# ZongyueQin/SessionSimilaritySearch

Hardware: AMD Instinct MI355X
Metric: session queries/sec (higher is better)
Workload: dtype f32

## Files before the change

sessionsimilaritysearch_amd/_lib.py:

```python
from __future__ import annotations

import ctypes
import os
import subprocess
from ctypes import c_float, c_int, c_int32, c_int64, c_size_t, c_void_p

_HERE = os.path.dirname(os.path.abspath(__file__))
LIB_PATH = os.path.join(_HERE, "libsss.so")
CSRC = os.path.join(_HERE, "csrc")

_lib = None

_SIGNATURES = {
    "sss_version": (c_int, []),
    "sss_last_error": (ctypes.c_char_p, []),
    "sss_normalize_rows": (c_int, [c_void_p, c_int64, c_int, c_int64, c_float, c_int, c_void_p]),
    "sss_row_norm_max": (c_int, [c_void_p, c_int64, c_int, c_int, c_void_p, c_void_p]),
    "sss_f32_to_bf16": (c_int, [c_void_p, c_int64, c_void_p, c_void_p]),
    "sss_ip_topk_workspace_bytes": (c_size_t, [c_int64, c_int64, c_int, c_int, c_int]),
    "sss_ip_topk_state_bytes": (c_size_t, [c_int64]),
    "sss_ip_topk": (c_int, [c_void_p, c_int64, c_void_p, c_int64, c_int, c_int, c_int, c_int64, c_float,
                            c_void_p, c_void_p, c_void_p, c_void_p, c_void_p, c_size_t, c_void_p, c_size_t, c_void_p]),
    "sss_split_bf16": (c_int, [c_void_p, c_int64, c_int, c_void_p, c_void_p]),
    "sss_ip_topk_split": (c_int, [c_void_p, c_int64, c_void_p, c_void_p, c_int64, c_int, c_int, c_int64, c_float,
# ... 84 lines not shown
    "sss_sparse_topk_workspace_bytes": (c_size_t, [c_int64, c_int64]),
    "sss_sparse_topk": (c_int, [c_void_p, c_void_p, c_void_p, c_int64, c_void_p, c_void_p, c_void_p, c_int64, c_int, c_int64,
                                c_void_p, c_void_p, c_void_p, c_size_t, c_void_p]),
}

_L2_SIGNATURES = {
    "sss_l2_row_bias": (c_int, [c_void_p, c_int64, c_int, c_void_p, c_void_p]),
    "sss_l2_topk_workspace_bytes": (c_size_t, [c_int64, c_int64, c_int, c_int, c_int]),
    "sss_l2_topk": (c_int, [c_void_p, c_int64, c_void_p, c_void_p, c_int, c_int, c_float, c_void_p, c_int64, c_int, c_int, c_int64,
                            c_float, c_void_p, c_void_p, c_void_p, c_void_p, c_void_p, c_size_t, c_void_p, c_size_t, c_void_p]),
    "sss_l2_topk_threshold_workspace_bytes": (c_size_t, [c_int64, c_int64, c_int, c_int]),
    "sss_l2_topk_threshold": (c_int, [c_void_p, c_void_p, c_int64, c_void_p, c_void_p, c_int, c_int, c_float, c_void_p, c_int64, c_int,
                                      c_int, c_int64, c_float, c_void_p, c_void_p, c_void_p, c_void_p, c_size_t, c_void_p]),
}


class LinearProblem(ctypes.Structure):
    _fields_ = [("x", c_void_p), ("ldx", c_int64), ("ids", c_void_p), ("table", c_void_p), ("xcopy", c_void_p),
                ("ld_xcopy", c_int64), ("w", c_void_p), ("ldw", c_int64), ("bias", c_void_p), ("y", c_void_p),
                ("ldy", c_int64), ("n", c_int64), ("m", c_int32), ("act", c_int32), ("post_scale", c_void_p), ("post_shift", c_void_p)]


class GraphOut(ctypes.Structure):
    _fields_ = [(n, c_void_p) for n in ("q_x", "q_batch", "q_pos", "p_x", "p_batch", "p_cnt", "rowptr_qp", "col_qp",
                                        "rowptr_pq", "col_pq", "rowptr_pp", "col_pp", "w_pp", "src_row", "pos_id")]


class LayerArgs(ctypes.Structure):
    _fields_ = [("yp", c_void_p), ("ld_yp", c_int64), ("yq", c_void_p), ("ld_yq", c_int64), ("h", c_int32), ("d_x", c_int32),
                ("rowptr_qp", c_void_p), ("col_qp", c_void_p), ("rowptr_pp", c_void_p), ("col_pp", c_void_p),
                ("w_pp", c_void_p), ("bias_qp", c_void_p), ("b_ih", c_void_p),
                ("xin_p", c_void_p), ("ld_xin", c_int64), ("out_p", c_void_p), ("ld_out_p", c_int64), ("np", c_int64),
                ("rowptr_pq", c_void_p), ("col_pq", c_void_p), ("bias_pq", c_void_p),
                ("out_q", c_void_p), ("ld_out_q", c_int64), ("nq", c_int64), ("n_self_loop", c_int64),
                ("row_p", c_void_p), ("row_q", c_void_p), ("x0_p", c_void_p), ("ld_x0_p", c_int64),
                ("xq_table", c_void_p), ("ld_xq", c_int64), ("x0_q", c_void_p), ("ld_x0_q", c_int64)]


def exported_symbols():
    return sorted(_SIGNATURES)


def sparse_symbols():
    return sorted(_SPARSE_SIGNATURES)


def l2_symbols():
    return sorted(_L2_SIGNATURES)


def build(verbose: bool = False) -> str:
    cmd = ["make", "-C", CSRC, "-j4"]
    res = subprocess.run(cmd, capture_output=True, text=True)
    if res.returncode != 0:
        raise RuntimeError("building libsss.so failed:\n" + res.stdout[-4000:] + res.stderr[-4000:])
    if verbose:
        print(res.stdout)
    return LIB_PATH


def lib():
    global _lib
    if _lib is None:
        if not os.path.exists(LIB_PATH):
            raise RuntimeError(
                f"{LIB_PATH} is missing: the HIP extension is not built. Run "
                "`python -c 'import __graft_entry__ as g; g.build()'` (or `make -C "
                "sessionsimilaritysearch_amd/csrc`). There is no CPU fallback.")
        h = ctypes.CDLL(LIB_PATH)
        for name, (res, args) in (*_SIGNATURES.items(), *_SPARSE_SIGNATURES.items(), *_L2_SIGNATURES.items()):
            fn = getattr(h, name)
            fn.restype, fn.argtypes = res, args
        _lib = h
    return _lib


class SssError(RuntimeError):
    pass


def check(rc: int, what: str):
    if rc != 0:
        msg = lib().sss_last_error()
        raise SssError(f"{what} failed (rc={rc}): {msg.decode() if msg else ''}")

# ... 16 lines not shown
```

sessionsimilaritysearch_amd/csrc/capi.hip:

```cpp
#include <stdarg.h>
#include <stdio.h>

#include <mutex>
#include <set>
#include <utility>

#include "../../include/sss.h"
#include "../../include/sss_sparse.h"
#include "../../include/sss_l2.h"
#include "sss_common.h"
#include "scan.h"
#include "kargs.h"

namespace sss {

static thread_local char g_err[512] = "";

void set_error(const char* fmt, ...) {
    va_list ap;
    va_start(ap, fmt);
    vsnprintf(g_err, sizeof(g_err), fmt, ap);
    va_end(ap);
}

// ... 34 lines not shown
int gather_concat_rows(const float*, const long*, int, const float*, long, int, int, long, float*, long, hipStream_t);
int linear_f32(const float*, long, const float*, long, const float*, float*, long, long, int, int, hipStream_t);
int gat_aggregate(const float*, long, const float*, long, const float*, long, const int*, const int*, long, int,
                  const float*, int, long, float*, long, hipStream_t);
int csr_weighted_sum(const float*, long, const int*, const int*, const float*, long, int, float*, long, hipStream_t);
int gru_combine(const float*, long, const float*, long, const float*, long, int, const float*, long, long, int,
                float*, long, hipStream_t);
int pool_expand(const float*, const float*, long, const int*, const int*, long, long, int, int, const float*, float*,
                long, hipStream_t);
int segment_pool(const float*, long, const int*, const int*, long, long, int, const float*, long, const float*, long,
                 const float*, float*, long, hipStream_t);
int segment_ptr(const long*, long, long, int*, hipStream_t);

int linear_grouped(LinBatch&, hipStream_t);
int layer_update(const LayerArgs&, hipStream_t);
int pool_expand_mean(const float*, const float*, long, const int*, const int*, const int*, const int*, long, long, int, int,
                     const float*, float*, long, float*, long, hipStream_t);
int pool_attention(const float*, long, const float*, long, const float*, long, const float*, const int*, const int*, long, long,
                   int, int, float, int, float*, long, hipStream_t);
int pool_attention_tab(const float*, long, const float*, long, const float*, const float*, const float*, const float*, const int*,
                       const int*, const int*, const int*, long, long, long, int, int, int, float, float*, long, hipStream_t);
int csr_mean(const float*, long, const int*, const int*, long, int, float*, long, hipStream_t);
int segment_reduce(const float*, long, const float*, const int*, long, int, int, float*, long, hipStream_t);
int attention_dot_pool(const float*, long, const int*, long, int, float*, long, hipStream_t);
int item_vote(const float*, const long*, long, int, const long*, const int*, long, long, int, long*, double*, int*, hipStream_t);
size_t hamming_workspace_bytes(long nq, long n);
int hamming_capacity(long nq, long n);
int hamming_topk(const unsigned char*, long, const unsigned char*, long, int, int, long, int*, long*, int*, void*, size_t, hipStream_t);
size_t hamming_exhaustive_workspace_bytes(long nsel, long n);
int hamming_topk_exhaustive(const unsigned char*, const int*, long, const unsigned char*, long, int, int, long, int*, long*, void*,
// ... 186 lines not shown
    sss::LinBatch b;
    b.nprob = n_problems; b.K = k;
    for (int i = 0; i < n_problems; ++i) {
        const sss_linear_problem& s = problems[i];
        sss::LinProb& p = b.p[i];
        p.x = s.x; p.ldx = s.ldx; p.ids = reinterpret_cast<const long*>(s.ids); p.table = s.table; p.xcopy = s.xcopy;
        p.ld_xcopy = s.ld_xcopy; p.w = s.w; p.ldw = s.ldw; p.bias = s.bias; p.y = s.y; p.ldy = s.ldy; p.n = s.n; p.m = s.m;
        p.act = s.act; p.post_scale = s.post_scale; p.post_shift = s.post_shift; p.tiles_m = 0; p.tile_begin = 0;
        if (s.act < 0 || s.act > 4 || (s.post_scale == nullptr) != (s.post_shift == nullptr)) {
            sss::set_error("linear_grouped: problem %d: act must be 0..4, post_scale / post_shift come together", i);
            return SSS_EINVAL;
        }
    }
    return sss::linear_grouped(b, ST(stream));
}
int sss_hetero_layer_update(const sss_layer_args* a, void* stream) {
    if (!a) { sss::set_error("hetero_layer_update: null args"); return SSS_EINVAL; }
    sss::LayerArgs l;
    l.Yp = a->yp; l.ldyp = a->ld_yp; l.Yq = a->yq; l.ldyq = a->ld_yq; l.h = a->h; l.d_x = a->d_x;
    l.rowptr_qp = a->rowptr_qp; l.col_qp = a->col_qp; l.rowptr_pp = a->rowptr_pp; l.col_pp = a->col_pp; l.w_pp = a->w_pp;
    l.bias_qp = a->bias_qp; l.b_ih = a->b_ih; l.xin_p = a->xin_p; l.ld_xin = a->ld_xin; l.out_p = a->out_p;
    l.ld_outp = a->ld_out_p; l.Np = a->np; l.rowptr_pq = a->rowptr_pq; l.col_pq = a->col_pq; l.bias_pq = a->bias_pq;
    l.out_q = a->out_q; l.ld_outq = a->ld_out_q; l.Nq = a->nq; l.n_self_loop = a->n_self_loop;
    l.row_p = reinterpret_cast<const long*>(a->row_p); l.row_q = reinterpret_cast<const long*>(a->row_q);
    l.x0_p = a->x0_p; l.ld_x0p = a->ld_x0_p; l.xq_table = a->xq_table; l.ld_xq = a->ld_xq; l.x0_q = a->x0_q; l.ld_x0q = a->ld_x0_q;
    return sss::layer_update(l, ST(stream));
}
int sss_pool_expand_mean(const float* lin_p, const float* lin_q, int64_t ld_lin, const int32_t* src_row,
                         const int32_t* pos_id, const int32_t* pptr, const int32_t* qptr, int64_t n_clicks,
                         int64_t n_graphs, int d_lin, int p, const float* pos_emb, float* node, int64_t ld_node,
                         float* coarse, int64_t ld_coarse, void* stream) {
    return sss::pool_expand_mean(lin_p, lin_q, ld_lin, src_row, pos_id, pptr, qptr, n_clicks, n_graphs, d_lin, p, pos_emb,
                                 node, ld_node, coarse, ld_coarse, ST(stream));
}
int sss_pool_attention(const float* node, int64_t ld_node, const float* a, int64_t ld_a, const float* b, int64_t ld_b,
                       const float* watt, const int32_t* pptr, const int32_t* qptr, int64_t n_clicks, int64_t n_graphs,
                       int d, int normalize, float eps, int reduce_sum, float* out, int64_t ld_out, void* stream) {
    return sss::pool_attention(node, ld_node, a, ld_a, b, ld_b, watt, pptr, qptr, n_clicks, n_graphs, d, normalize, eps,
                               reduce_sum, out, ld_out, ST(stream));
}
int sss_pool_attention_tab(const float* t, int64_t ld_t, const float* ac, int64_t ld_ac, const float* tanhpos, const float* a2tab,
// ... 50 lines not shown
    g.rowptr_qp = o->rowptr_qp; g.col_qp = o->col_qp; g.rowptr_pq = o->rowptr_pq; g.col_pq = o->col_pq;
    g.rowptr_pp = o->rowptr_pp; g.col_pp = o->col_pp; g.w_pp = o->w_pp; g.src_row = o->src_row; g.pos_id = o->pos_id;
    return sss::graph_fill(reinterpret_cast<const long*>(sess_ptr), is_search, reinterpret_cast<const long*>(item_id),
                           reinterpret_cast<const long*>(query_tok), n_sessions, bases, g, ST(stream));
}
int sss_knn_item_vote(const float* D, const int64_t* I, int64_t nq, int s, const int64_t* items_ptr, const int32_t* items,
                      int64_t id_offset, int64_t n_sessions, int k, int64_t* out_items, double* out_weights,
                      int32_t* status, void* stream) {
    return sss::item_vote(D, reinterpret_cast<const long*>(I), nq, s, reinterpret_cast<const long*>(items_ptr), items,
                          id_offset, n_sessions, k, reinterpret_cast<long*>(out_items), out_weights, status, ST(stream));
}
int sss_segment_ptr(const int64_t* batch, int64_t n, int64_t n_graphs, int32_t* ptr, void* stream) {
    return sss::segment_ptr(reinterpret_cast<const long*>(batch), n, n_graphs, ptr, ST(stream));
}

int sss_session_vectors_count(const int64_t* sess_ptr, const uint8_t* is_search, const int64_t* item_id, int64_t n_sessions,
                              int64_t n_items, int32_t* counts, int32_t* err, void* stream) {
    return sss::session_vectors_count(reinterpret_cast<const long*>(sess_ptr), is_search, reinterpret_cast<const long*>(item_id),
                                      n_sessions, n_items, counts, err, ST(stream));
}
int sss_session_vectors_fill(const int64_t* sess_ptr, const uint8_t* is_search, const int64_t* item_id, int64_t n_sessions,
                             int64_t n_items, int mode, double lammy, const int64_t* ptr, int32_t* items, float* weights,
                             int32_t* err, void* stream) {
    return sss::session_vectors_fill(reinterpret_cast<const long*>(sess_ptr), is_search, reinterpret_cast<const long*>(item_id),
                                     n_sessions, n_items, mode, lammy, reinterpret_cast<const long*>(ptr), items, weights, err,
                                     ST(stream));
}
size_t sss_sparse_topk_workspace_bytes(int64_t nq, int64_t n) { return sss::sparse_topk_workspace_bytes(nq, n); }
int sss_sparse_topk(const int64_t* q_ptr, const int32_t* q_items, const float* q_weights, int64_t nq, const int64_t* c_ptr,
                    const int32_t* c_items, const float* c_weights, int64_t n, int k, int64_t id_offset, float* D_out,
// ... 32 lines not shown
```

sessionsimilaritysearch_amd/csrc/gnn.hip:

```cpp
#include "sss_common.h"
#include "kargs.h"

namespace sss {

int normalize_rows(float* x, long n, int d, long ld, float eps, int rule, hipStream_t st);

constexpr int LT = 64;

int linear_grouped(LinBatch& b, hipStream_t st);

template <int LPR>
__global__ __launch_bounds__(256) void k_gat_aggregate(
    const float* __restrict__ xs, long ld_xs, const float* __restrict__ a_src, long ld_as,
    const float* __restrict__ a_dst, long ld_ad, const int* __restrict__ rowptr,
    const int* __restrict__ col, long n_dst, int h, const float* __restrict__ bias, int relu,
    long n_self_loop, float* __restrict__ out, long ld_out) {
    const int sub = threadIdx.x % LPR;
    const long per_block = 256 / LPR;
    const int nv = h / 4;
    auto score = [&](long j, float ad) {
        const float v = a_src[j * ld_as] + ad;
        return v > 0.f ? v : 0.2f * v;
    };
    for (long i = (long)blockIdx.x * per_block + threadIdx.x / LPR; i < n_dst; i += (long)gridDim.x * per_block) {
// ... 326 lines not shown
                                           out, ld_out));
    return check_launch("k_segment_pool");
}

int segment_ptr(const long* batch, long n, long n_graphs, int* ptr, hipStream_t st) {
    if (n < 0 || n_graphs < 0) { set_error("segment_ptr: bad arguments"); return SSS_EINVAL; }
    hipLaunchKernelGGL(k_segment_ptr, dim3((unsigned)((n_graphs + 1 + 255) / 256)), dim3(256), 0, st, batch, n, n_graphs, ptr);
    return check_launch("k_segment_ptr");
}

}

namespace sss {


template <int KC>
__global__ __launch_bounds__(256, 2) void k_linear_grouped(const LinBatch B) {
    constexpr int CPR = KC / 4;
    constexpr int NLD = LT * CPR / 256;
    constexpr int RS = CPR;
    constexpr int SW = RS < 16 ? RS - 1 : 15;
    extern __shared__ __attribute__((aligned(16))) float lds_raw[];
    float* lx = lds_raw;
    float* lw = lds_raw + LT * RS * 4;
    int pi = 0;
#pragma unroll
    for (int i = 1; i < 4; ++i)
        if (i < B.nprob && (int)blockIdx.x >= B.p[i].tile_begin) pi = i;
    const float* X = B.p[0].x; long ldx = B.p[0].ldx; const long* ids = B.p[0].ids; const float* table = B.p[0].table;
    float* xcopy = B.p[0].xcopy; long ldc = B.p[0].ld_xcopy; const float* W = B.p[0].w; long ldw = B.p[0].ldw;
    const float* bias = B.p[0].bias; float* Y = B.p[0].y; long ldy = B.p[0].ldy; long N = B.p[0].n; int M = B.p[0].m;
    int tiles_m = B.p[0].tiles_m, tile_begin = B.p[0].tile_begin, act = B.p[0].act;
    const float* post_s = B.p[0].post_scale; const float* post_t = B.p[0].post_shift;
#pragma unroll
    for (int i = 1; i < 4; ++i)
        if (pi == i) {
            act = B.p[i].act; post_s = B.p[i].post_scale; post_t = B.p[i].post_shift;
            X = B.p[i].x; ldx = B.p[i].ldx; ids = B.p[i].ids; table = B.p[i].table; xcopy = B.p[i].xcopy; ldc = B.p[i].ld_xcopy;
            W = B.p[i].w; ldw = B.p[i].ldw; bias = B.p[i].bias; Y = B.p[i].y; ldy = B.p[i].ldy; N = B.p[i].n; M = B.p[i].m;
            tiles_m = B.p[i].tiles_m; tile_begin = B.p[i].tile_begin;
        }
    const int K = B.K;
    const int t = (int)blockIdx.x - tile_begin;
    const long row0 = (long)(t / tiles_m) * LT;
    const int col0 = (t % tiles_m) * LT;
    const int tid = threadIdx.x, lane = tid & 63, wave = tid >> 6;
    const int wr = wave >> 1, wc = wave & 1;
    const int r = lane & 31, h = lane >> 5;
    const int xr = wr * 32 + r, wrow = wc * 32 + r;

    f32x16 acc = {0};
    f32x4 sx[NLD], sw[NLD];
    auto fetch = [&](int k0) {
#pragma unroll
        for (int i = 0; i < NLD; ++i) {
            const int p = tid + 256 * i;
            const int tr = p / CPR, c = p % CPR;
            long gr = row0 + tr; if (gr > N - 1) gr = N - 1;
            int gw = col0 + tr; if (gw > M - 1) gw = M - 1;
            const float* xrow = ids ? table + ids[gr] * (long)K : X + gr * ldx;
            sx[i] = *reinterpret_cast<const f32x4*>(xrow + k0 + c * 4);
// ... 35 lines not shown
    if (col < M) {
        const float bv = bias ? bias[col] : 0.f;
        const float ps = post_s ? post_s[col] : 1.f, pt = post_s ? post_t[col] : 0.f;
#pragma unroll
        for (int j = 0; j < 16; ++j) {
            const long row = row0 + wr * 32 + (j & 3) + 8 * (j >> 2) + 4 * h;
            float v = acc[j] + bv;
            if (act == 1) v = fmaxf(v, 0.f);
            else if (act == 2) v = tanhf(v);
            else if (act == 3) v = v > 0.f ? 1.f : v < 0.f ? -1.f : v;
            else if (act == 4) v = tanhf(tanhf(v));
            if (post_s) {
#pragma clang fp contract(off)
                v = fmaxf(v * ps + pt, 0.f);
            }
            if (row < N) Y[row * ldy + col] = v;
        }
    }
}


__device__ __forceinline__ float4 f4_fma(float w, float4 x, float4 a) {
    a.x += w * x.x; a.y += w * x.y; a.z += w * x.z; a.w += w * x.w;
    return a;
}
__device__ __forceinline__ float leaky02(float v) { return v > 0.f ? v : 0.2f * v; }

__device__ __forceinline__ float4 gat_row(const float* xs, long ld, const float* a_src_col, float ad, const int* col,
                                          int e0, int e1, int c4, const float* bias, long skip_i, long self_i,
                                          const long* row_of = nullptr) {
    float mx = -INFINITY, den = 0.f;
    float4 acc = make_float4(0.f, 0.f, 0.f, 0.f);
    auto edge = [&](long jn) {
// ... 7 lines not shown
        }
        const float ex = expf(v - mx);
        den += ex;
        acc = f4_fma(ex, x, acc);
    };
    for (int e = e0; e < e1; ++e) {
        const long j = col[e];
        if (j != skip_i) edge(j);
    }
    if (self_i >= 0) edge(self_i);
    const float inv = 1.f / (den + 1e-16f);
    const float4 b = *reinterpret_cast<const float4*>(bias + c4);
    return make_float4(acc.x * inv + b.x, acc.y * inv + b.y, acc.z * inv + b.z, acc.w * inv + b.w);
}

template <int LPR>
__global__ __launch_bounds__(256) void k_layer_update(const LayerArgs A) {
    const int sub = threadIdx.x % LPR;
    const long per_block = 256 / LPR;
    const long t = (long)blockIdx.x * per_block + threadIdx.x / LPR;
    const int h = A.h, c4 = sub * 4;
    if (c4 >= h || t >= A.Np + A.Nq) return;
    if (t >= A.Np) {
        const long i = t - A.Np;
        const long ri = A.row_q ? A.row_q[i] : i;
        const float ad = A.Yq[ri * A.ldyq + h + 1];
        const bool lp = i < A.n_self_loop;
        float4 o = gat_row(A.Yp, A.ldyp, A.Yp + 7 * h, ad, A.col_pq, A.rowptr_pq[i], A.rowptr_pq[i + 1], c4, A.bias_pq,
                           A.n_self_loop > 0 ? i : -1, lp ? i : -1, A.row_p);
        if (A.x0_q) {
            const float* xq = A.xq_table + ri * A.ld_xq;
            float* dq = A.x0_q + i * A.ld_x0q;
            if (c4 + 3 < A.d_x) *reinterpret_cast<float4*>(dq + c4) = *reinterpret_cast<const float4*>(xq + c4);
            else for (int u = 0; u < 4; ++u) if (c4 + u < A.d_x) dq[c4 + u] = xq[c4 + u];
        }
        o.x = fmaxf(o.x, 0.f); o.y = fmaxf(o.y, 0.f); o.z = fmaxf(o.z, 0.f); o.w = fmaxf(o.w, 0.f);
        *reinterpret_cast<float4*>(A.out_q + i * A.ld_outq + c4) = o;
// ... 34 lines not shown
            if (c4 + 1 < A.d_x) dp[c4 + 1] = xv.y;
            if (c4 + 2 < A.d_x) dp[c4 + 2] = xv.z;
        }
    }
    float4 o;
#define SSS_GRU1(f)                                                        \
    {                                                                      \
        const float rr = sigmoidf_(gr.f + hr.f);                           \
        const float zz = sigmoidf_(gz.f + hz.f);                           \
        const float nn = tanhf(gn.f + rr * hn.f);                          \
        o.f = fmaxf(t1.f + (1.f - zz) * nn + zz * xv.f, 0.f);              \
    }
    SSS_GRU1(x) SSS_GRU1(y) SSS_GRU1(z) SSS_GRU1(w)
#undef SSS_GRU1
    *reinterpret_cast<float4*>(A.out_p + i * A.ld_outp + c4) = o;
}

template <int LPR>
__global__ __launch_bounds__(256) void k_pool_expand_mean(const float* __restrict__ lin_p, const float* __restrict__ lin_q,
                                                          long ld_lin, const int* __restrict__ src_row,
                                                          const int* __restrict__ pos_id, const int* __restrict__ pptr,
                                                          const int* __restrict__ qptr, long n_clicks, long n_graphs,
                                                          int Dl, int P, const float* __restrict__ pos_emb,
                                                          float* __restrict__ node, long ld_node,
                                                          float* __restrict__ coarse, long ld_coarse) {
    const int sub = threadIdx.x % LPR;
    const long g = (long)blockIdx.x * (256 / LPR) + threadIdx.x / LPR;
    const int D = Dl + P, c4 = sub * 4;
    if (g >= n_graphs || c4 >= D) return;
    const int p0 = pptr[g], p1 = pptr[g + 1], q0 = qptr[g], q1 = qptr[g + 1];
// ... 186 lines not shown
            (p.ids && (!p.table || (p.xcopy && (p.ld_xcopy % 4 || p.ld_xcopy < b.K))))) {
            set_error("linear_grouped: problem %d has bad strides / shapes", i);
            return SSS_EINVAL;
        }
        p.tiles_m = (p.m + LT - 1) / LT;
        p.tile_begin = total;
        total += (int)((p.n + LT - 1) / LT) * p.tiles_m;
    }
    for (int i = b.nprob; i < 4; ++i) { b.p[i] = b.p[0]; b.p[i].tile_begin = 0x7fffffff; }
    if (total == 0) return SSS_OK;
    const int lds32 = 2 * LT * 8 * 16;
    hipLaunchKernelGGL(k_linear_grouped<32>, dim3((unsigned)total), dim3(256), lds32, st, b);
    return check_launch("k_linear_grouped");
}

int layer_update(const LayerArgs& a, hipStream_t st) {
    if (a.h <= 0 || a.h % 4 || a.h > 256 || a.Np < 0 || a.Nq < 0 || a.d_x > a.h || a.ldyp % 4 || a.ldyq % 4 || a.ld_outp % 4 ||
        a.ld_outq % 4 || (a.d_x >= 4 && a.ld_xin % 4) || a.ldyp < 7 * a.h + 2 || a.ldyq < a.h + 2) {
        set_error("layer_update: need h %% 4 == 0, h <= 256, d_x <= h, 16-byte aligned row strides, ldyp >= 7h+2, ldyq >= h+2");
        return SSS_EINVAL;
    }
    if ((a.x0_p && a.ld_x0p % 4) || (a.x0_q && (!a.xq_table || a.ld_xq % 4 || a.ld_x0q % 4))) {
        set_error("layer_update: x0_p / x0_q need 16-byte aligned row strides, x0_q needs xq_table");
        return SSS_EINVAL;
    }
    const long total = a.Np + a.Nq;
    if (total == 0) return SSS_OK;
    const int lpr = lanes_for(a.h);
    const long per = 256 / lpr;
    SSS_LPR_SWITCH(lpr, hipLaunchKernelGGL(k_layer_update<L>, dim3((unsigned)((total + per - 1) / per)), dim3(256), 0, st, a));
    return check_launch("k_layer_update");
}

int pool_expand_mean(const float* lin_p, const float* lin_q, long ld_lin, const int* src_row, const int* pos_id,
                     const int* pptr, const int* qptr, long n_clicks, long n_graphs, int Dl, int P, const float* pos_emb,
                     float* node, long ld_node, float* coarse, long ld_coarse, hipStream_t st) {
    const int D = Dl + P;
    if (n_graphs < 0 || Dl <= 0 || P < 0 || D % 4 || D > 256 || ld_node % 4 || ld_node < D || ld_coarse % 4 || ld_coarse < D) {
        set_error("pool_expand_mean: need (Dl + P) %% 4 == 0, <= 256, 16-byte aligned row strides");
        return SSS_EINVAL;
    }
    if (n_graphs == 0) return SSS_OK;
    const int lpr = lanes_for(D);
    const long per = 256 / lpr;
    SSS_LPR_SWITCH(lpr, hipLaunchKernelGGL(k_pool_expand_mean<L>, dim3((unsigned)((n_graphs + per - 1) / per)), dim3(256), 0, st,
                                           lin_p, lin_q, ld_lin, src_row, pos_id, pptr, qptr, n_clicks, n_graphs, Dl, P, pos_emb,
// ... 47 lines not shown
```

sessionsimilaritysearch_amd/csrc/kargs.h:

```cpp
#pragma once
#include "sss_common.h"

namespace sss {

struct LinProb {
    const float* x; long ldx;
    const long* ids; const float* table;
    float* xcopy; long ld_xcopy;
    const float* w; long ldw; const float* bias;
    float* y; long ldy;
    long n; int m;
    int act;
    const float* post_scale = nullptr;
    const float* post_shift = nullptr;
    int tiles_m, tile_begin;
};
struct LinBatch { LinProb p[4]; int nprob; int K; };

struct LayerArgs {
    const float* Yp; long ldyp; const float* Yq; long ldyq; int h;
    const int* rowptr_qp; const int* col_qp; const int* rowptr_pp; const int* col_pp; const float* w_pp;
    const float* bias_qp; const float* b_ih; const float* xin_p; long ld_xin; int d_x; float* out_p; long ld_outp; long Np;
    const int* rowptr_pq; const int* col_pq; const float* bias_pq; float* out_q; long ld_outq; long Nq;
    long n_self_loop;
    const long* row_p = nullptr; const long* row_q = nullptr;
    float* x0_p = nullptr; long ld_x0p = 0;
    const float* xq_table = nullptr; long ld_xq = 0; float* x0_q = nullptr; long ld_x0q = 0;
};

struct GraphOut {
    long* q_x; long* q_batch; int* q_pos;
    long* p_x; long* p_batch; long* p_cnt;
    int* rowptr_qp; int* col_qp;
    int* rowptr_pq; int* col_pq;
    int* rowptr_pp; int* col_pp; float* w_pp;
    int* src_row; int* pos_id;
};

}
```

sessionsimilaritysearch_amd/encoder.py:

```python
from __future__ import annotations

import ctypes
import itertools
import math
from dataclasses import dataclass

import numpy as np
import torch

from . import _lib
from .sessions import ASIN_NUM, EDGE_PP, EDGE_PQ, EDGE_QP, MAX_SEQ_LEN, QUERY_VOCAB, ActionTable

ALPHA_PAD = 32


@dataclass
class EncoderConfig:
    d_in: int = 128
    d_id: int = 0
    h: int = 128
    n_layers: int = 2
    d_out: int = 128
    max_seq_len: int = MAX_SEQ_LEN
    n_items: int = ASIN_NUM
# ... 94 lines not shown
    rowptr[1:] = torch.cumsum(counts, 0).to(torch.int32)
    wv = None if w is None else w[order].float().contiguous()
    return rowptr, col, wv


class PreparedBatch:
    """Device-resident batch: feature ids + CSR adjacencies + pooling index arrays
    (``SessionEncoder.prepare``)."""


class SessionEncoder:

    _serials = itertools.count()

    def __init__(self, cfg: EncoderConfig, weights: dict, device=None, use_edge_weight: bool = False,
                 debug_nan_checks: bool = False, fused: bool = True):
        cfg.validate()
        self._serial = next(SessionEncoder._serials)
        if not torch.cuda.is_available():
            raise _lib.SssError("no HIP device available: the encoder runs on MI355X only")
        _lib.lib()
        self.user_cfg = cfg
        self.d_id, self.d_feat = cfg.d_id, cfg.d_in
        if cfg.d_id:
            weights = self._internal_weights(cfg, weights)
            cfg = EncoderConfig(**{**cfg.__dict__, "d_in": cfg.d_p, "d_id": 0})
        self.cfg = cfg
        self.device = torch.device("cuda", torch.cuda.current_device()) if device is None else torch.device(device)
        self.use_edge_weight = use_edge_weight
        self.debug_nan_checks = debug_nan_checks
        self.fused = fused
        self.training = False
        self._prepare(weights)

    def eval(self):
        self.training = False
        return self

    def to(self, device):
        if torch.device(device) != self.device:
            raise _lib.SssError("SessionEncoder is bound to its construction device")
        return self

    def __call__(self, *a, **kw):
        return self.forward(*a, **kw)

# ... 267 lines not shown
                self._tabs = ()
            else:
                Yp = torch.empty((ni, 7 * h + ALPHA_PAD), dtype=torch.float32, device=self.device)
                Yq = torch.empty((nqy, h + ALPHA_PAD), dtype=torch.float32, device=self.device)
                P_ = _lib.LinearProblem
                mk = lambda x, w, b, y, n, m: P_(x=x.data_ptr(), ldx=x.stride(0), ids=0, table=0, xcopy=0, ld_xcopy=0,
                                                 w=w.data_ptr(), ldw=w.stride(0), bias=0 if b is None else b.data_ptr(),
                                                 y=y.data_ptr(), ldy=y.stride(0), n=n, m=m, act=0)
                arr = (P_ * 2)(mk(self.item_table, lw["w7"], lw["b7"], Yp, ni, 7 * h + 2),
                               mk(self.query_table, lw["wq"], None, Yq, nqy, h + 2))
                _lib.check(_lib.lib().sss_linear_grouped(arr, 2, lw["din"], self._st()), "sss_linear_grouped")
                self._tabs = (Yp, Yq)
        return self._tabs or None

    def _fused_calls(self, pb, ws, gather):
        key = "gather" if gather else "rows"
        if key in ws["calls"]:
            return ws["calls"][key]
        cfg = self.cfg
        h, D, P, W = cfg.h, cfg.d_out, cfg.max_seq_len, cfg.node_width
        NQ, NP, Yp, Yq = ws["NQ"], ws["NP"], ws["Yp"], ws["Yq"]
        P_ = _lib.LinearProblem

        def prob(x, w, bias, y, n, m, ids=None, table=None, xcopy=None):
            return P_(x=0 if x is None else x.data_ptr(), ldx=0 if x is None else x.stride(0),
                      ids=0 if ids is None else ids.data_ptr(), table=0 if table is None else table.data_ptr(),
                      xcopy=0 if xcopy is None else xcopy.data_ptr(), ld_xcopy=0 if xcopy is None else xcopy.stride(0),
                      w=w.data_ptr(), ldw=w.stride(0), bias=0 if bias is None else bias.data_ptr(),
                      y=y.data_ptr(), ldy=y.stride(0), n=n, m=m, act=0)

        steps, keep = [], []
# ... 28 lines not shown
                                np=pb.Np, rowptr_pq=rp_pq.data_ptr(), col_pq=c_pq.data_ptr(),
                                bias_pq=lw["bias_pq"].data_ptr(), out_q=out_q.data_ptr(), ld_out_q=NQ.stride(0), nq=pb.Nq,
                                n_self_loop=pb.n_self_loop,
                                row_p=pb.p_ids.data_ptr() if table0 else 0, row_q=pb.q_ids.data_ptr() if table0 else 0,
                                x0_p=NP.data_ptr() if table0 else 0, ld_x0_p=NP.stride(0),
                                xq_table=self.query_table.data_ptr() if table0 else 0,
                                ld_xq=self.query_table.stride(0) if table0 else 0,
                                x0_q=NQ.data_ptr() if table0 else 0, ld_x0_q=NQ.stride(0))
            if arr is not None:
                steps.append(("lin", arr, 2, din))
            steps.append(("layer", la))
            keep += [arr, la]
        pw, pt = self.pool, self.pool_tab
        Dl = D - P
        T, AC = ws["T"], ws["AC"]
        pp, pq = prob(NP, pw["wp"], pw["bp"], T[:pb.Np], pb.Np, Dl), prob(NQ, pw["wq"], pw["bq"], T[pb.Np:], pb.Nq, Dl)
        pp.act = pq.act = 2
        arr = (P_ * 2)(pp, pq)
        steps.append(("lin", arr, 2, W))
        arr2 = (P_ * 1)(prob(T, pt["wnc"], None, AC, pb.Np + pb.Nq, 2 * D))
        steps.append(("lin", arr2, 1, pt["KT"]))
        ws["calls"][key] = steps
        return steps

    def _forward_fused(self, pb, get_node, query_node_mask, product_node_mask, l2_normalize):
        cfg, L, dev = self.cfg, _lib.lib(), self.device
        h, D, P, W = cfg.h, cfg.d_out, cfg.max_seq_len, cfg.node_width
        ws = self._workspace(pb, get_node)
        NQ, NP = ws["NQ"], ws["NP"]
        masked = query_node_mask is not None or product_node_mask is not None
        gather = pb.q_feat is None and pb.p_feat is None and not masked
        if not gather:
            self._features(pb.q_ids, pb.q_feat, self.query_table, pb.Nq, NQ)
            self._features(pb.p_ids, pb.p_feat, self.item_table, pb.Np, NP, product=True)
            if query_node_mask is not None:
                NQ[:, :cfg.d_in] *= query_node_mask.to(dev, torch.float32).view(-1, 1)
            if product_node_mask is not None:
                NP[:, :cfg.d_in] *= product_node_mask.to(dev, torch.float32).view(-1, 1)
        elif self.item_table is None or self.query_table is None:
            raise _lib.SssError("no feature table in the weights and no .feat on the batch")
        st = self._st()
        pw = self.pool
        for step in self._fused_calls(pb, ws, gather):
            if step[0] == "lin":
                _lib.check(L.sss_linear_grouped(step[1], step[2], step[3], st), "sss_linear_grouped")
            else:
                _lib.check(L.sss_hetero_layer_update(ctypes.byref(step[1]), st), "sss_hetero_layer_update")
        out = torch.empty((pb.B, D), dtype=torch.float32, device=dev)
        pt, T, AC = self.pool_tab, ws["T"], ws["AC"]
        rc = L.sss_pool_attention_tab(T.data_ptr(), T.stride(0), AC.data_ptr(), AC.stride(0), pt["tanhpos"].data_ptr(),
                                      pt["a2"].data_ptr(), pt["c2"].data_ptr(), pw["watt"].data_ptr(), pb.src_row.data_ptr(),
                                      pb.pos_id.data_ptr(), pb.pptr.data_ptr(), pb.qptr.data_ptr(), pb.n_clicks, pb.Np, pb.B,
                                      D - P, P, 1 if l2_normalize else 0, 1e-6, out.data_ptr(), D, st)
        _lib.check(rc, "sss_pool_attention_tab")
        return out, NQ, NP

    @torch.no_grad()
    def forward(self, data, query_node_mask=None, product_node_mask=None, get_node=False, get_token=False,
                l2_normalize=False):
        cfg, L, dev = self.cfg, _lib.lib(), self.device
        h, D, P, W = cfg.h, cfg.d_out, cfg.max_seq_len, cfg.node_width
        pb = self.prepare(data)
# ... 90 lines not shown
```

Before: 487,200.

## Fuse last GNN layer update with pooling-head linear projections in one kernel

Adds a kernel that, per 64-row tile, runs the final hetero layer GRU update, then the per-type pooling projection (tanh) into T, then the wnc projection into AC, using 1024-thread blocks of four 256-thread teams. The three launches become one, and each tile's intermediates stay L2/LDS-local instead of round-tripping between launches. The linear tile body is refactored into a shared device function. The cost is fewer blocks (one per row tile), with teams idling when the column tile count isn't a multiple of four, and a smaller K chunk of 32, which could reduce GEMM efficiency.

```diff
diff --git a/include/sss_encoder.h b/include/sss_encoder.h
--- /dev/null
+++ b/include/sss_encoder.h
@@ -0,0 +1,22 @@
+#ifndef SSS_ENCODER_H
+#define SSS_ENCODER_H
+
+#include "sss.h"
+
+#ifdef __cplusplus
+extern "C" {
+#endif
+
+typedef struct {
+    const float* node_p; int64_t ld_np; const float* node_q; int64_t ld_nq; int32_t node_width;
+    const float* wp; int64_t ld_wp; const float* bp; const float* wq; int64_t ld_wq; const float* bq; int32_t d_lin;
+    float* t; int64_t ld_t; int32_t kt;
+    const float* wnc; int64_t ld_wnc; float* ac; int64_t ld_ac; int32_t m_ac;
+} sss_head_args;
+
+int sss_layer_update_head(const sss_layer_args* layer, const sss_head_args* head, void* stream);
+
+#ifdef __cplusplus
+}
+#endif
+#endif
diff --git a/sessionsimilaritysearch_amd/_lib.py b/sessionsimilaritysearch_amd/_lib.py
--- a/sessionsimilaritysearch_amd/_lib.py
+++ b/sessionsimilaritysearch_amd/_lib.py
@@ -122,6 +122,10 @@
                                       c_int, c_int64, c_float, c_void_p, c_void_p, c_void_p, c_void_p, c_size_t, c_void_p]),
 }
 
+_ENCODER_SIGNATURES = {
+    "sss_layer_update_head": (c_int, [c_void_p, c_void_p, c_void_p]),
+}
+
 
 class LinearProblem(ctypes.Structure):
     _fields_ = [("x", c_void_p), ("ldx", c_int64), ("ids", c_void_p), ("table", c_void_p), ("xcopy", c_void_p),
@@ -145,6 +149,13 @@
                 ("xq_table", c_void_p), ("ld_xq", c_int64), ("x0_q", c_void_p), ("ld_x0_q", c_int64)]
 
 
+class HeadArgs(ctypes.Structure):
+    _fields_ = [("node_p", c_void_p), ("ld_np", c_int64), ("node_q", c_void_p), ("ld_nq", c_int64), ("node_width", c_int32),
+                ("wp", c_void_p), ("ld_wp", c_int64), ("bp", c_void_p), ("wq", c_void_p), ("ld_wq", c_int64), ("bq", c_void_p),
+                ("d_lin", c_int32), ("t", c_void_p), ("ld_t", c_int64), ("kt", c_int32),
+                ("wnc", c_void_p), ("ld_wnc", c_int64), ("ac", c_void_p), ("ld_ac", c_int64), ("m_ac", c_int32)]
+
+
 def exported_symbols():
     return sorted(_SIGNATURES)
 
@@ -155,6 +166,10 @@
 
 def l2_symbols():
     return sorted(_L2_SIGNATURES)
+
+
+def encoder_symbols():
+    return sorted(_ENCODER_SIGNATURES)
 
 
 def build(verbose: bool = False) -> str:
@@ -176,7 +191,8 @@
                 "`python -c 'import __graft_entry__ as g; g.build()'` (or `make -C "
                 "sessionsimilaritysearch_amd/csrc`). There is no CPU fallback.")
         h = ctypes.CDLL(LIB_PATH)
-        for name, (res, args) in (*_SIGNATURES.items(), *_SPARSE_SIGNATURES.items(), *_L2_SIGNATURES.items()):
+        for name, (res, args) in (*_SIGNATURES.items(), *_SPARSE_SIGNATURES.items(), *_L2_SIGNATURES.items(),
+                                  *_ENCODER_SIGNATURES.items()):
             fn = getattr(h, name)
             fn.restype, fn.argtypes = res, args
         _lib = h
diff --git a/sessionsimilaritysearch_amd/csrc/capi.hip b/sessionsimilaritysearch_amd/csrc/capi.hip
--- a/sessionsimilaritysearch_amd/csrc/capi.hip
+++ b/sessionsimilaritysearch_amd/csrc/capi.hip
@@ -8,6 +8,7 @@
 #include "../../include/sss.h"
 #include "../../include/sss_sparse.h"
 #include "../../include/sss_l2.h"
+#include "../../include/sss_encoder.h"
 #include "sss_common.h"
 #include "scan.h"
 #include "kargs.h"
@@ -72,6 +73,7 @@
 
 int linear_grouped(LinBatch&, hipStream_t);
 int layer_update(const LayerArgs&, hipStream_t);
+int layer_update_head(const LayerArgs&, const HeadArgs&, hipStream_t);
 int pool_expand_mean(const float*, const float*, long, const int*, const int*, const int*, const int*, long, long, int, int,
                      const float*, float*, long, float*, long, hipStream_t);
 int pool_attention(const float*, long, const float*, long, const float*, long, const float*, const int*, const int*, long, long,
@@ -288,8 +290,7 @@
     }
     return sss::linear_grouped(b, ST(stream));
 }
-int sss_hetero_layer_update(const sss_layer_args* a, void* stream) {
-    if (!a) { sss::set_error("hetero_layer_update: null args"); return SSS_EINVAL; }
+static sss::LayerArgs layer_args(const sss_layer_args* a) {
     sss::LayerArgs l;
     l.Yp = a->yp; l.ldyp = a->ld_yp; l.Yq = a->yq; l.ldyq = a->ld_yq; l.h = a->h; l.d_x = a->d_x;
     l.rowptr_qp = a->rowptr_qp; l.col_qp = a->col_qp; l.rowptr_pp = a->rowptr_pp; l.col_pp = a->col_pp; l.w_pp = a->w_pp;
@@ -298,7 +299,11 @@
     l.out_q = a->out_q; l.ld_outq = a->ld_out_q; l.Nq = a->nq; l.n_self_loop = a->n_self_loop;
     l.row_p = reinterpret_cast<const long*>(a->row_p); l.row_q = reinterpret_cast<const long*>(a->row_q);
     l.x0_p = a->x0_p; l.ld_x0p = a->ld_x0_p; l.xq_table = a->xq_table; l.ld_xq = a->ld_xq; l.x0_q = a->x0_q; l.ld_x0q = a->ld_x0_q;
-    return sss::layer_update(l, ST(stream));
+    return l;
+}
+int sss_hetero_layer_update(const sss_layer_args* a, void* stream) {
+    if (!a) { sss::set_error("hetero_layer_update: null args"); return SSS_EINVAL; }
+    return sss::layer_update(layer_args(a), ST(stream));
 }
 int sss_pool_expand_mean(const float* lin_p, const float* lin_q, int64_t ld_lin, const int32_t* src_row,
                          const int32_t* pos_id, const int32_t* pptr, const int32_t* qptr, int64_t n_clicks,
@@ -379,6 +384,16 @@
     return sss::segment_ptr(reinterpret_cast<const long*>(batch), n, n_graphs, ptr, ST(stream));
 }
 
+int sss_layer_update_head(const sss_layer_args* a, const sss_head_args* hd, void* stream) {
+    if (!a || !hd) { sss::set_error("layer_update_head: null args"); return SSS_EINVAL; }
+    sss::HeadArgs h;
+    h.node_p = hd->node_p; h.ld_np = hd->ld_np; h.node_q = hd->node_q; h.ld_nq = hd->ld_nq; h.W = hd->node_width;
+    h.wp = hd->wp; h.ldwp = hd->ld_wp; h.bp = hd->bp; h.wq = hd->wq; h.ldwq = hd->ld_wq; h.bq = hd->bq; h.Dl = hd->d_lin;
+    h.T = hd->t; h.ld_t = hd->ld_t; h.KT = hd->kt; h.wnc = hd->wnc; h.ld_wnc = hd->ld_wnc; h.AC = hd->ac; h.ld_ac = hd->ld_ac;
+    h.M_ac = hd->m_ac;
+    return sss::layer_update_head(layer_args(a), h, ST(stream));
+}
+
 int sss_session_vectors_count(const int64_t* sess_ptr, const uint8_t* is_search, const int64_t* item_id, int64_t n_sessions,
                               int64_t n_items, int32_t* counts, int32_t* err, void* stream) {
     return sss::session_vectors_count(reinterpret_cast<const long*>(sess_ptr), is_search, reinterpret_cast<const long*>(item_id),
diff --git a/sessionsimilaritysearch_amd/csrc/gnn.hip b/sessionsimilaritysearch_amd/csrc/gnn.hip
--- a/sessionsimilaritysearch_amd/csrc/gnn.hip
+++ b/sessionsimilaritysearch_amd/csrc/gnn.hip
@@ -364,37 +364,24 @@
 namespace sss {
 
 
+struct LinTile {
+    const float* X; long ldx; const long* ids; const float* table; float* xcopy; long ldc;
+    const float* W; long ldw; const float* bias; float* Y; long ldy; long N; int M; int act;
+    const float* post_s; const float* post_t;
+};
+
 template <int KC>
-__global__ __launch_bounds__(256, 2) void k_linear_grouped(const LinBatch B) {
+__device__ __forceinline__ void linear_tile(float* lx, float* lw, const LinTile& P, const int K, const long row0,
+                                            const int col0, const int tid, const bool store) {
     constexpr int CPR = KC / 4;
     constexpr int NLD = LT * CPR / 256;
     constexpr int RS = CPR;
     constexpr int SW = RS < 16 ? RS - 1 : 15;
-    extern __shared__ __attribute__((aligned(16))) float lds_raw[];
-    float* lx = lds_raw;
-    float* lw = lds_raw + LT * RS * 4;
-    int pi = 0;
-#pragma unroll
-    for (int i = 1; i < 4; ++i)
-        if (i < B.nprob && (int)blockIdx.x >= B.p[i].tile_begin) pi = i;
-    const float* X = B.p[0].x; long ldx = B.p[0].ldx; const long* ids = B.p[0].ids; const float* table = B.p[0].table;
-    float* xcopy = B.p[0].xcopy; long ldc = B.p[0].ld_xcopy; const float* W = B.p[0].w; long ldw = B.p[0].ldw;
-    const float* bias = B.p[0].bias; float* Y = B.p[0].y; long ldy = B.p[0].ldy; long N = B.p[0].n; int M = B.p[0].m;
-    int tiles_m = B.p[0].tiles_m, tile_begin = B.p[0].tile_begin, act = B.p[0].act;
-    const float* post_s = B.p[0].post_scale; const float* post_t = B.p[0].post_shift;
-#pragma unroll
-    for (int i = 1; i < 4; ++i)
-        if (pi == i) {
-            act = B.p[i].act; post_s = B.p[i].post_scale; post_t = B.p[i].post_shift;
-            X = B.p[i].x; ldx = B.p[i].ldx; ids = B.p[i].ids; table = B.p[i].table; xcopy = B.p[i].xcopy; ldc = B.p[i].ld_xcopy;
-            W = B.p[i].w; ldw = B.p[i].ldw; bias = B.p[i].bias; Y = B.p[i].y; ldy = B.p[i].ldy; N = B.p[i].n; M = B.p[i].m;
-            tiles_m = B.p[i].tiles_m; tile_begin = B.p[i].tile_begin;
-        }
-    const int K = B.K;
-    const int t = (int)blockIdx.x - tile_begin;
-    const long row0 = (long)(t / tiles_m) * LT;
-    const int col0 = (t % tiles_m) * LT;
-    const int tid = threadIdx.x, lane = tid & 63, wave = tid >> 6;
+    const float* X = P.X; const long ldx = P.ldx; const long* ids = P.ids; const float* table = P.table;
+    float* xcopy = P.xcopy; const long ldc = P.ldc; const float* W = P.W; const long ldw = P.ldw;
+    const float* bias = P.bias; float* Y = P.Y; const long ldy = P.ldy; const long N = P.N; const int M = P.M;
+    const int act = P.act; const float* post_s = P.post_s; const float* post_t = P.post_t;
+    const int lane = tid & 63, wave = tid >> 6;
     const int wr = wave >> 1, wc = wave & 1;
     const int r = lane & 31, h = lane >> 5;
     const int xr = wr * 32 + r, wrow = wc * 32 + r;
@@ -460,9 +447,33 @@
 #pragma clang fp contract(off)
                 v = fmaxf(v * ps + pt, 0.f);
             }
-            if (row < N) Y[row * ldy + col] = v;
-        }
-    }
+            if (row < N && store) Y[row * ldy + col] = v;
+        }
+    }
+}
+
+template <int KC>
+__global__ __launch_bounds__(256, 2) void k_linear_grouped(const LinBatch B) {
+    extern __shared__ __attribute__((aligned(16))) float lds_raw[];
+    float* lx = lds_raw;
+    float* lw = lds_raw + LT * KC;
+    int pi = 0;
+#pragma unroll
+    for (int i = 1; i < 4; ++i)
+        if (i < B.nprob && (int)blockIdx.x >= B.p[i].tile_begin) pi = i;
+    LinTile P = {B.p[0].x, B.p[0].ldx, B.p[0].ids, B.p[0].table, B.p[0].xcopy, B.p[0].ld_xcopy, B.p[0].w, B.p[0].ldw,
+                 B.p[0].bias, B.p[0].y, B.p[0].ldy, B.p[0].n, B.p[0].m, B.p[0].act, B.p[0].post_scale, B.p[0].post_shift};
+    int tiles_m = B.p[0].tiles_m, tile_begin = B.p[0].tile_begin;
+#pragma unroll
+    for (int i = 1; i < 4; ++i)
+        if (pi == i) {
+            P.act = B.p[i].act; P.post_s = B.p[i].post_scale; P.post_t = B.p[i].post_shift;
+            P.X = B.p[i].x; P.ldx = B.p[i].ldx; P.ids = B.p[i].ids; P.table = B.p[i].table; P.xcopy = B.p[i].xcopy; P.ldc = B.p[i].ld_xcopy;
+            P.W = B.p[i].w; P.ldw = B.p[i].ldw; P.bias = B.p[i].bias; P.Y = B.p[i].y; P.ldy = B.p[i].ldy; P.N = B.p[i].n; P.M = B.p[i].m;
+            tiles_m = B.p[i].tiles_m; tile_begin = B.p[i].tile_begin;
+        }
+    const int t = (int)blockIdx.x - tile_begin;
+    linear_tile<KC>(lx, lw, P, B.K, (long)(t / tiles_m) * LT, (t % tiles_m) * LT, (int)threadIdx.x, true);
 }
 
 
@@ -500,13 +511,8 @@
     return make_float4(acc.x * inv + b.x, acc.y * inv + b.y, acc.z * inv + b.z, acc.w * inv + b.w);
 }
 
-template <int LPR>
-__global__ __launch_bounds__(256) void k_layer_update(const LayerArgs A) {
-    const int sub = threadIdx.x % LPR;
-    const long per_block = 256 / LPR;
-    const long t = (long)blockIdx.x * per_block + threadIdx.x / LPR;
-    const int h = A.h, c4 = sub * 4;
-    if (c4 >= h || t >= A.Np + A.Nq) return;
+__device__ __forceinline__ void layer_update_node(const LayerArgs& A, const long t, const int c4) {
+    const int h = A.h;
     if (t >= A.Np) {
         const long i = t - A.Np;
         const long ri = A.row_q ? A.row_q[i] : i;
@@ -571,6 +577,63 @@
     SSS_GRU1(x) SSS_GRU1(y) SSS_GRU1(z) SSS_GRU1(w)
 #undef SSS_GRU1
     *reinterpret_cast<float4*>(A.out_p + i * A.ld_outp + c4) = o;
+}
+
+template <int LPR>
+__global__ __launch_bounds__(256) void k_layer_update(const LayerArgs A) {
+    const int sub = threadIdx.x % LPR;
+    const long per_block = 256 / LPR;
+    const long t = (long)blockIdx.x * per_block + threadIdx.x / LPR;
+    const int c4 = sub * 4;
+    if (c4 >= A.h || t >= A.Np + A.Nq) return;
+    layer_update_node(A, t, c4);
+}
+
+constexpr int HEAD_TEAMS = 4;
+constexpr int HEAD_KC = 32;
+
+template <int LPR>
+__global__ __launch_bounds__(256 * HEAD_TEAMS) void k_layer_update_head(const LayerArgs A, const HeadArgs H) {
+    extern __shared__ __attribute__((aligned(16))) float lds_raw[];
+    const int tid = threadIdx.x & 255, team = threadIdx.x >> 8;
+    float* lx = lds_raw + team * (2 * LT * HEAD_KC);
+    float* lw = lx + LT * HEAD_KC;
+    const long blocks_p = (A.Np + LT - 1) / LT;
+    const bool isq = (long)blockIdx.x >= blocks_p;
+    const long row0 = ((long)blockIdx.x - (isq ? blocks_p : 0)) * LT;
+    const long n_type = isq ? A.Nq : A.Np, t0 = isq ? A.Np : 0;
+    {
+        const int c4 = ((int)threadIdx.x % LPR) * 4;
+        constexpr int PER = 256 * HEAD_TEAMS / LPR;
+        if (c4 < A.h)
+            for (int r = (int)threadIdx.x / LPR; r < LT; r += PER)
+                if (row0 + r < n_type) layer_update_node(A, t0 + row0 + r, c4);
+    }
+    __threadfence_block();
+    __syncthreads();
+    {
+        const LinTile P = {isq ? H.node_q : H.node_p, isq ? H.ld_nq : H.ld_np, nullptr, nullptr, nullptr, 0,
+                           isq ? H.wq : H.wp, isq ? H.ldwq : H.ldwp, isq ? H.bq : H.bp, H.T + t0 * H.ld_t, H.ld_t,
+                           n_type, H.Dl, 2, nullptr, nullptr};
+        const int tiles_m = (H.Dl + LT - 1) / LT;
+        for (int c0 = 0; c0 < tiles_m; c0 += HEAD_TEAMS) {
+            const int ct = c0 + team;
+            if (c0 > 0) __syncthreads();
+            linear_tile<HEAD_KC>(lx, lw, P, H.W, row0, (ct < tiles_m ? ct : tiles_m - 1) * LT, tid, ct < tiles_m);
+        }
+    }
+    __threadfence_block();
+    __syncthreads();
+    {
+        const LinTile P = {H.T + t0 * H.ld_t, H.ld_t, nullptr, nullptr, nullptr, 0, H.wnc, H.ld_wnc, nullptr,
+                           H.AC + t0 * H.ld_ac, H.ld_ac, n_type, H.M_ac, 0, nullptr, nullptr};
+        const int tiles_m = (H.M_ac + LT - 1) / LT;
+        for (int c0 = 0; c0 < tiles_m; c0 += HEAD_TEAMS) {
+            const int ct = c0 + team;
+            if (c0 > 0) __syncthreads();
+            linear_tile<HEAD_KC>(lx, lw, P, H.KT, row0, (ct < tiles_m ? ct : tiles_m - 1) * LT, tid, ct < tiles_m);
+        }
+    }
 }
 
 template <int LPR>
@@ -787,7 +850,7 @@
     return check_launch("k_linear_grouped");
 }
 
-int layer_update(const LayerArgs& a, hipStream_t st) {
+static int check_layer_args(const LayerArgs& a) {
     if (a.h <= 0 || a.h % 4 || a.h > 256 || a.Np < 0 || a.Nq < 0 || a.d_x > a.h || a.ldyp % 4 || a.ldyq % 4 || a.ld_outp % 4 ||
         a.ld_outq % 4 || (a.d_x >= 4 && a.ld_xin % 4) || a.ldyp < 7 * a.h + 2 || a.ldyq < a.h + 2) {
         set_error("layer_update: need h %% 4 == 0, h <= 256, d_x <= h, 16-byte aligned row strides, ldyp >= 7h+2, ldyq >= h+2");
@@ -797,12 +860,33 @@
         set_error("layer_update: x0_p / x0_q need 16-byte aligned row strides, x0_q needs xq_table");
         return SSS_EINVAL;
     }
+    return SSS_OK;
+}
+
+int layer_update(const LayerArgs& a, hipStream_t st) {
+    if (const int rc = check_layer_args(a)) return rc;
     const long total = a.Np + a.Nq;
     if (total == 0) return SSS_OK;
     const int lpr = lanes_for(a.h);
     const long per = 256 / lpr;
     SSS_LPR_SWITCH(lpr, hipLaunchKernelGGL(k_layer_update<L>, dim3((unsigned)((total + per - 1) / per)), dim3(256), 0, st, a));
     return check_launch("k_layer_update");
+}
+
+int layer_update_head(const LayerArgs& a, const HeadArgs& hd, hipStream_t st) {
+    if (const int rc = check_layer_args(a)) return rc;
+    if (hd.W <= 0 || hd.W % 32 || hd.KT <= 0 || hd.KT % 32 || hd.Dl <= 0 || hd.Dl > hd.KT || hd.M_ac <= 0 ||
+        hd.ld_np % 4 || hd.ld_np < hd.W || hd.ld_nq % 4 || hd.ld_nq < hd.W || hd.ldwp % 4 || hd.ldwp < hd.W || hd.ldwq % 4 ||
+        hd.ldwq < hd.W || hd.ld_t % 4 || hd.ld_t < hd.KT || hd.ld_wnc % 4 || hd.ld_wnc < hd.KT || hd.ld_ac < hd.M_ac) {
+        set_error("layer_update_head: need W %% 32 == 0, KT %% 32 == 0, Dl <= KT, 16-byte aligned row strides >= the row widths");
+        return SSS_EINVAL;
+    }
+    const long blocks = (a.Np + LT - 1) / LT + (a.Nq + LT - 1) / LT;
+    if (blocks == 0) return SSS_OK;
+    const int lpr = lanes_for(a.h);
+    const int lds = HEAD_TEAMS * 2 * LT * HEAD_KC * 4;
+    SSS_LPR_SWITCH(lpr, hipLaunchKernelGGL(k_layer_update_head<L>, dim3((unsigned)blocks), dim3(256 * HEAD_TEAMS), lds, st, a, hd));
+    return check_launch("k_layer_update_head");
 }
 
 int pool_expand_mean(const float* lin_p, const float* lin_q, long ld_lin, const int* src_row, const int* pos_id,
diff --git a/sessionsimilaritysearch_amd/csrc/kargs.h b/sessionsimilaritysearch_amd/csrc/kargs.h
--- a/sessionsimilaritysearch_amd/csrc/kargs.h
+++ b/sessionsimilaritysearch_amd/csrc/kargs.h
@@ -28,6 +28,13 @@
     const float* xq_table = nullptr; long ld_xq = 0; float* x0_q = nullptr; long ld_x0q = 0;
 };
 
+struct HeadArgs {
+    const float* node_p; long ld_np; const float* node_q; long ld_nq; int W;
+    const float* wp; long ldwp; const float* bp; const float* wq; long ldwq; const float* bq; int Dl;
+    float* T; long ld_t; int KT;
+    const float* wnc; long ld_wnc; float* AC; long ld_ac; int M_ac;
+};
+
 struct GraphOut {
     long* q_x; long* q_batch; int* q_pos;
     long* p_x; long* p_batch; long* p_cnt;
diff --git a/sessionsimilaritysearch_amd/encoder.py b/sessionsimilaritysearch_amd/encoder.py
--- a/sessionsimilaritysearch_amd/encoder.py
+++ b/sessionsimilaritysearch_amd/encoder.py
@@ -132,7 +132,7 @@
     _serials = itertools.count()
 
     def __init__(self, cfg: EncoderConfig, weights: dict, device=None, use_edge_weight: bool = False,
-                 debug_nan_checks: bool = False, fused: bool = True):
+                 debug_nan_checks: bool = False, fused: bool = True, fuse_head: bool = True):
         cfg.validate()
         self._serial = next(SessionEncoder._serials)
         if not torch.cuda.is_available():
@@ -148,6 +148,7 @@
         self.use_edge_weight = use_edge_weight
         self.debug_nan_checks = debug_nan_checks
         self.fused = fused
+        self.fuse_head = fuse_head
         self.training = False
         self._prepare(weights)
 
@@ -445,7 +446,8 @@
         return self._tabs or None
 
     def _fused_calls(self, pb, ws, gather):
-        key = "gather" if gather else "rows"
+        head = self.fuse_head and bool(self.layers)
+        key = ("gather" if gather else "rows") + ("+head" if head else "")
         if key in ws["calls"]:
             return ws["calls"][key]
         cfg = self.cfg
@@ -504,12 +506,21 @@
         pw, pt = self.pool, self.pool_tab
         Dl = D - P
         T, AC = ws["T"], ws["AC"]
-        pp, pq = prob(NP, pw["wp"], pw["bp"], T[:pb.Np], pb.Np, Dl), prob(NQ, pw["wq"], pw["bq"], T[pb.Np:], pb.Nq, Dl)
-        pp.act = pq.act = 2
-        arr = (P_ * 2)(pp, pq)
-        steps.append(("lin", arr, 2, W))
-        arr2 = (P_ * 1)(prob(T, pt["wnc"], None, AC, pb.Np + pb.Nq, 2 * D))
-        steps.append(("lin", arr2, 1, pt["KT"]))
+        if head:
+            _, la = steps.pop()
+            ha = _lib.HeadArgs(node_p=NP.data_ptr(), ld_np=NP.stride(0), node_q=NQ.data_ptr(), ld_nq=NQ.stride(0), node_width=W,
+                               wp=pw["wp"].data_ptr(), ld_wp=pw["wp"].stride(0), bp=pw["bp"].data_ptr(),
+                               wq=pw["wq"].data_ptr(), ld_wq=pw["wq"].stride(0), bq=pw["bq"].data_ptr(), d_lin=Dl,
+                               t=T.data_ptr(), ld_t=T.stride(0), kt=pt["KT"], wnc=pt["wnc"].data_ptr(),
+                               ld_wnc=pt["wnc"].stride(0), ac=AC.data_ptr(), ld_ac=AC.stride(0), m_ac=2 * D)
+            steps.append(("head", la, ha))
+        else:
+            pp, pq = prob(NP, pw["wp"], pw["bp"], T[:pb.Np], pb.Np, Dl), prob(NQ, pw["wq"], pw["bq"], T[pb.Np:], pb.Nq, Dl)
+            pp.act = pq.act = 2
+            arr = (P_ * 2)(pp, pq)
+            steps.append(("lin", arr, 2, W))
+            arr2 = (P_ * 1)(prob(T, pt["wnc"], None, AC, pb.Np + pb.Nq, 2 * D))
+            steps.append(("lin", arr2, 1, pt["KT"]))
         ws["calls"][key] = steps
         return steps
 
@@ -534,8 +545,10 @@
         for step in self._fused_calls(pb, ws, gather):
             if step[0] == "lin":
                 _lib.check(L.sss_linear_grouped(step[1], step[2], step[3], st), "sss_linear_grouped")
+            elif step[0] == "layer":
+                _lib.check(L.sss_hetero_layer_update(ctypes.byref(step[1]), st), "sss_hetero_layer_update")
             else:
-                _lib.check(L.sss_hetero_layer_update(ctypes.byref(step[1]), st), "sss_hetero_layer_update")
+                _lib.check(L.sss_layer_update_head(ctypes.byref(step[1]), ctypes.byref(step[2]), st), "sss_layer_update_head")
         out = torch.empty((pb.B, D), dtype=torch.float32, device=dev)
         pt, T, AC = self.pool_tab, ws["T"], ws["AC"]
         rc = L.sss_pool_attention_tab(T.data_ptr(), T.stride(0), AC.data_ptr(), AC.stride(0), pt["tanhpos"].data_ptr(),
```

After: 482,900. Within noise of the previous version (-0.9%).
